# jimahlstrom/quisk

Measured on AMD Instinct MI355X. Metric: Mcomplex-samples/s through RXA chain, higher is better.
Workload: dtype f64; 1 GPU; 256 channels/GPU x 192 kHz IQ -> 48 kHz SSB RXA chain (shift + 561-tap resample/4 + adc meter + NBP nc 2048 + S meter + fixed AGC + agc meter + panel), 2^22 input samples per channel per step; meters=on, ingest=f64, channels_per_gpu=256, total_channels=256, dsp_size=256, parallelism=channel-sharded x1 (weak), no collective

## Files before the change

### quisk_amd/csrc/qh_fft.hpp

```cpp
#pragma once
#include <hip/hip_runtime.h>

namespace qh {

static constexpr double kThetaZeroMark = 8.0;


constexpr int NT = 256;

template <typename T> struct cplx_of;
template <> struct cplx_of<double> { using type = double2; };
template <> struct cplx_of<float>  { using type = float2; };
template <typename T> using cplx = typename cplx_of<T>::type;

template <typename T> __device__ __forceinline__ cplx<T> mk(T x, T y) { cplx<T> r; r.x = x; r.y = y; return r; }
template <typename C> __device__ __forceinline__ C cadd(C a, C b) { C r; r.x = a.x + b.x; r.y = a.y + b.y; return r; }
template <typename C> __device__ __forceinline__ C csub(C a, C b) { C r; r.x = a.x - b.x; r.y = a.y - b.y; return r; }
template <typename C> __device__ __forceinline__ C cmul(C a, C b)
{
    C r;
    r.x = a.x * b.x - a.y * b.y;
    r.y = a.x * b.y + a.y * b.x;
    return r;
}
__device__ __forceinline__ void lds_barrier()
{
    __builtin_amdgcn_fence(__ATOMIC_RELEASE, "workgroup", "local");
    __builtin_amdgcn_s_barrier();
    __builtin_amdgcn_fence(__ATOMIC_ACQUIRE, "workgroup", "local");
}

template <typename C> __device__ __forceinline__ C cconj(C a) { C r; r.x = a.x; r.y = -a.y; return r; }
template <bool INV, typename C> __device__ __forceinline__ C mul_mi(C a)
{
    C r;
    if (INV) { r.x = -a.y; r.y = a.x; } else { r.x = a.y; r.y = -a.x; }
    return r;
}

__device__ __forceinline__ constexpr double cos32(int a)
{
    constexpr double t[9] = { 1.0, 0.98078528040323044913, 0.92387953251128675613, 0.83146961230254523708,
                              0.70710678118654752440, 0.55557023301960222474, 0.38268343236508977173,
                              0.19509032201612826785, 0.0 };
    return t[a];
}

template <int R, int I, bool INV, typename C> __device__ __forceinline__ C mul_wconst(C a)
{
    using T = decltype(a.x);
    constexpr int A = I * (32 / R);
    if constexpr (A == 0) {
        return a;
    } else if constexpr (A == 8) {
        return mul_mi<INV>(a);
    } else if constexpr (A == 4) {
        const T s = (T)0.70710678118654752440;
        C r;
        if (INV) { r.x = (a.x - a.y) * s; r.y = (a.x + a.y) * s; }
        else     { r.x = (a.x + a.y) * s; r.y = (a.y - a.x) * s; }
        return r;
    } else if constexpr (A == 12) {
        const T s = (T)0.70710678118654752440;
        C r;
        if (INV) { r.x = -(a.x + a.y) * s; r.y = (a.x - a.y) * s; }
        else     { r.x = (a.y - a.x) * s;  r.y = -(a.x + a.y) * s; }
        return r;
    } else {
        constexpr double c = (A <= 8) ? cos32(A) : -cos32(16 - A);
        constexpr double s = (A <= 8) ? cos32(8 - A) : cos32(A - 8);
        C w;
        w.x = (T)c;
        w.y = INV ? (T)s : (T)(-s);
        return cmul(a, w);
    }
}

template <int R, bool INV, typename C> struct Dft {
    template <int I> static __device__ __forceinline__ void stage(C (&x)[R], C (&a)[R / 2], C (&b)[R / 2])
    {
        if constexpr (I < R / 2) {
            a[I] = cadd(x[I], x[I + R / 2]);
            b[I] = mul_wconst<R, I, INV>(csub(x[I], x[I + R / 2]));
            stage<I + 1>(x, a, b);
        }
    }
    static __device__ __forceinline__ void run(C (&x)[R])
    {
        C a[R / 2], b[R / 2];
        stage<0>(x, a, b);
        Dft<R / 2, INV, C>::run(a);
        Dft<R / 2, INV, C>::run(b);
#pragma unroll
        for (int q = 0; q < R / 2; q++) { x[2 * q] = a[q]; x[2 * q + 1] = b[q]; }
    }
};
template <bool INV, typename C> struct Dft<1, INV, C> { static __device__ __forceinline__ void run(C (&)[1]) {} };

__device__ __forceinline__ int lds_phys(int i) { return i + (i >> 4); }
template <int N> constexpr int lds_elems() { return N + N / 16; }

template <int R, typename C> __device__ __forceinline__ void apply_twiddle_powers(C (&x)[R], C w1)
{
    constexpr int H = R / 2 > 1 ? R / 2 : 1;
    C w[H + 1];
    w[1] = w1;
    x[1] = cmul(x[1], w1);
#pragma unroll
    for (int r = 2; r < R; r++) {
        int hi = 1;
        while (hi * 2 <= r) hi *= 2;
        const int lo = r - hi;
        C wr;
        if (hi < H || (hi == H && lo == 0)) {
            wr = (lo == 0) ? cmul(w[hi / 2], w[hi / 2]) : cmul(w[hi], w[lo]);
            w[r < H + 1 ? r : H] = wr;
        } else {
            wr = cmul(w[H], w[lo]);
        }
        x[r] = cmul(x[r], wr);
    }
}

template <int R, typename C> __device__ __forceinline__ void apply_twiddle_powers_lean(C (&x)[R], C w1)
{
    const C w2 = cmul(w1, w1);
    C we = w2, wo = w1;
    x[1] = cmul(x[1], wo);
#pragma unroll
    for (int r = 2; r < R; r++) {
        if (r & 1) { wo = cmul(wo, w2); x[r] = cmul(x[r], wo); }
        else { x[r] = cmul(x[r], we); if (r + 2 < R) we = cmul(we, w2); }
    }
}

template <int N, int R, int Ns, bool INV, typename C, bool LEAN = false>
__device__ __forceinline__ int stockham_butterfly(C (&x)[R], int j, C w1)
{
    int k = j & (Ns - 1);
    if constexpr (Ns > 1) { if constexpr (LEAN) apply_twiddle_powers_lean<R>(x, w1); else apply_twiddle_powers<R>(x, w1); }
    Dft<R, INV, C>::run(x);
    return (j - k) * R + k;
}

template <int Ns, bool INV, typename C>
__device__ __forceinline__ C pass_twiddle(const C *__restrict__ tw_pass, int j)
{
    C w = tw_pass[j & (Ns - 1)];
    return INV ? cconj(w) : w;
}

template <int N, int R, bool INV, typename C>
__device__ __forceinline__ void pass_regs_to_lds(C (&x)[R], C *lds)
{
    static_assert(R == N / NT, "first pass radix must equal N/NT");
    const int j = threadIdx.x;
    Dft<R, INV, C>::run(x);
    if constexpr (16 % R == 0) {
        C *p = lds + lds_phys(j * R);
#pragma unroll
        for (int r = 0; r < R; r++) p[r] = x[r];
    } else {
        static_assert(R % 16 == 0, "first pass radix: a divisor or a multiple of 16");
        C *p = lds + lds_phys(j * R);
#pragma unroll
        for (int r = 0; r < R; r++) p[r + r / 16] = x[r];
    }
}

template <int N, int R> struct PassGeom {
    static constexpr int NB = N / R;
    static constexpr int PER = (NB + NT - 1) / NT;
};

template <int N, int R, int Ns, bool INV, typename C>
__device__ __forceinline__ void pass_lds_to_lds(C *lds, const C (&w1)[PassGeom<N, R>::PER])
{
    constexpr int NB = PassGeom<N, R>::NB;
    constexpr int PER = PassGeom<N, R>::PER;
    C x[PER][R];
    int base[PER];
    static_assert(NB % 16 == 0, "pass geometry");
#pragma unroll
    for (int p = 0; p < PER; p++) {
        int j = threadIdx.x + p * NT;
        if (NB >= NT || j < NB) {
            const C *q = lds + lds_phys(j);
#pragma unroll
            for (int r = 0; r < R; r++) x[p][r] = q[r * (NB + NB / 16)];
        }
    }
#pragma unroll
    for (int p = 0; p < PER; p++) {
        int j = threadIdx.x + p * NT;
        if (NB >= NT || j < NB) base[p] = stockham_butterfly<N, R, Ns, INV>(x[p], j, w1[p]);
    }
    __syncthreads();
#pragma unroll
    for (int p = 0; p < PER; p++) {
        int j = threadIdx.x + p * NT;
        if (NB >= NT || j < NB) {
            if constexpr (Ns % 16 == 0) {
                C *q = lds + lds_phys(base[p]);
#pragma unroll
                for (int r = 0; r < R; r++) q[r * (Ns + Ns / 16)] = x[p][r];
            } else if constexpr (16 % (Ns * R) == 0) {
                C *q = lds + lds_phys(base[p]);
#pragma unroll
                for (int r = 0; r < R; r++) q[r * Ns] = x[p][r];
            } else {
#pragma unroll
                for (int r = 0; r < R; r++) lds[lds_phys(base[p] + r * Ns)] = x[p][r];
            }
        }
    }
}

template <int N, int R, bool INV, typename C>
__device__ __forceinline__ void pass_lds_to_regs(const C *lds, C (&x)[R], C w1)
{
    static_assert(R == N / NT, "last pass radix must equal N/NT");
    const int j = threadIdx.x;
    const C *q = lds + lds_phys(j);
#pragma unroll
    for (int r = 0; r < R; r++) x[r] = q[r * (NT + NT / 16)];
    stockham_butterfly<N, R, N / R, INV>(x, j, w1);
}

template <int N, bool INV, typename C> struct FftRR;

template <bool INV, typename C> struct FftRR<4096, INV, C> {
    struct Tw { C a[1], b; };
    static __device__ __forceinline__ Tw load(const C *__restrict__ tw) { return load_at(tw, threadIdx.x); }
    static __device__ __forceinline__ Tw load_at(const C *__restrict__ tw, int j)
    {
        Tw t;
        t.a[0] = pass_twiddle<16, INV>(tw, j);
        t.b = pass_twiddle<256, INV>(tw + 16, j);
        return t;
    }
    static __device__ __forceinline__ void first(C (&x)[16], C *lds) { pass_regs_to_lds<4096, 16, INV>(x, lds); }
    static __device__ __forceinline__ void rest(C *lds, C (&x)[16], const Tw &t)
    {
        __syncthreads();
        pass_lds_to_lds<4096, 16, 16, INV>(lds, t.a);
        __syncthreads();
        pass_lds_to_regs<4096, 16, INV>(lds, x, t.b);
    }
};

#ifndef QH_SPLIT_PAD
#define QH_SPLIT_PAD 2
#endif
#ifndef QH_SPLIT_SWIZZLE
#define QH_SPLIT_SWIZZLE 0
#endif
constexpr int split4096_lds_bytes(int scalar_bytes) { return (QH_SPLIT_SWIZZLE ? 4096 : 4096 + QH_SPLIT_PAD * 256) * scalar_bytes; }
template <bool INV, typename C> struct FftSplit4096 {
    using T = decltype(C{}.x);
    using Tw = typename FftRR<4096, INV, C>::Tw;
    static constexpr bool kSwizzle = QH_SPLIT_SWIZZLE != 0;
    template <int PHASE>
    static __device__ __forceinline__ void exchange_sw(C (&x)[16], T *lds, int j, int base)
    {
        const int m = j & 15;
        T *wb = PHASE == 1 ? lds + 16 * j : lds + (base - m);
        const T *rp = lds + 16 * (j >> 4) + (m ^ ((j >> 4) & 15));
#pragma unroll
        for (int r = 0; r < 16; r++) (PHASE == 1 ? wb : wb + 16 * r)[PHASE == 1 ? (r ^ m) : (m ^ r)] = x[r].x;
        __syncthreads();
#pragma unroll
        for (int r = 0; r < 16; r++) x[r].x = rp[256 * r];
        __syncthreads();
#pragma unroll
        for (int r = 0; r < 16; r++) (PHASE == 1 ? wb : wb + 16 * r)[PHASE == 1 ? (r ^ m) : (m ^ r)] = x[r].y;
        __syncthreads();
#pragma unroll
        for (int r = 0; r < 16; r++) x[r].y = rp[256 * r];
    }
    static constexpr int kPad = QH_SPLIT_PAD;
    static constexpr int kLdsBytes = split4096_lds_bytes((int)sizeof(T));
    static __device__ __forceinline__ int sphys(int i) { return i + (i >> 4) * kPad; }

    template <int WS, int RS, bool LB = false>
    static __device__ __forceinline__ void exchange(C (&x)[16], T *lds, int wbase, int rbase)
    {
        T *wp = lds + wbase;
        const T *rp = lds + rbase;
#pragma unroll
        for (int r = 0; r < 16; r++) wp[r * WS] = x[r].x;
        if (LB) lds_barrier(); else __syncthreads();
#pragma unroll
        for (int r = 0; r < 16; r++) x[r].x = rp[r * RS];
        if (LB) lds_barrier(); else __syncthreads();
#pragma unroll
        for (int r = 0; r < 16; r++) wp[r * WS] = x[r].y;
        if (LB) lds_barrier(); else __syncthreads();
#pragma unroll
        for (int r = 0; r < 16; r++) x[r].y = rp[r * RS];
    }

    static __device__ __forceinline__ void run(C (&x)[16], void *lds_raw, const Tw &t) { run_at(x, lds_raw, t, threadIdx.x); }
    template <bool LEAN = false>
    static __device__ __forceinline__ void run_at(C (&x)[16], void *lds_raw, const Tw &t, int j)
    {
        T *lds = reinterpret_cast<T *>(lds_raw);
        Dft<16, INV, C>::run(x);
        if constexpr (kSwizzle) exchange_sw<1>(x, lds, j, 0);
        else exchange<1, 256 + 16 * kPad>(x, lds, (16 + kPad) * j, sphys(j));
        const int base = stockham_butterfly<4096, 16, 16, INV, C, LEAN>(x, j, t.a[0]);
        __syncthreads();
        if constexpr (kSwizzle) exchange_sw<2>(x, lds, j, base);
        else exchange<16 + kPad, 256 + 16 * kPad>(x, lds, sphys(base), sphys(j));
        stockham_butterfly<4096, 16, 256, INV, C, LEAN>(x, j, t.b);
    }

    template <int D>
    static __device__ __forceinline__ void run_poly(C (&x)[16], void *lds_raw, const Tw &t)
    {
        static_assert(!INV && (D == 2 || D == 4 || D == 8), "forward transform of a decimating stage");
        constexpr int R3 = 16 / D;
        const int j = threadIdx.x;
        T *lds = reinterpret_cast<T *>(lds_raw);
        Dft<16, INV, C>::run(x);
        if constexpr (kSwizzle) exchange_sw<1>(x, lds, j, 0);
        else exchange<1, 256 + 16 * kPad>(x, lds, (16 + kPad) * j, sphys(j));
        const int base = stockham_butterfly<4096, 16, 16, INV>(x, j, t.a[0]);
        __syncthreads();
        if constexpr (kSwizzle) exchange_sw<2>(x, lds, j, base);
        else exchange<16 + kPad, 256 + 16 * kPad>(x, lds, sphys(base), sphys(j));
        C w[R3];
        w[1] = t.b;
#pragma unroll
        for (int s = 1; s < D; s <<= 1) w[1] = cmul(w[1], w[1]);
#pragma unroll
        for (int r = 2; r < R3; r++) w[r] = (r & 1) ? cmul(w[r - 1], w[1]) : cmul(w[r / 2], w[r / 2]);
        C y[16];
#pragma unroll
        for (int a = 0; a < D; a++) {
            C b[R3];
            b[0] = x[a];
#pragma unroll
            for (int r = 1; r < R3; r++) b[r] = cmul(x[a + D * r], w[r]);
            Dft<R3, INV, C>::run(b);
#pragma unroll
            for (int r = 0; r < R3; r++) y[r + R3 * a] = b[r];
        }
#pragma unroll
        for (int r = 0; r < 16; r++) x[r] = y[r];
    }
};

constexpr int kFft6kThreads = 384;
constexpr int kFft6kPad = 2;
constexpr int kFft6kLdsBytes = (6144 + 6144 / 16 * kFft6kPad) * 8;

template <bool INV, typename C> __device__ __forceinline__ void dft3(C &a, C &b, C &c)
{
    const double h = 0.86602540378443864676;
    const C t1 = cadd(b, c);
    C t2; t2.x = a.x - 0.5 * t1.x; t2.y = a.y - 0.5 * t1.y;
    const C d = csub(b, c);
    C t3;
    if (INV) { t3.x = -h * d.y; t3.y = h * d.x; } else { t3.x = h * d.y; t3.y = -h * d.x; }
    a = cadd(a, t1);
    b = cadd(t2, t3);
    c = csub(t2, t3);
}

template <int M, bool INV, typename C> __device__ __forceinline__ C mul_w24(C a)
{
    constexpr int m = M % 24;
    if constexpr (m == 0) return a;
    else if constexpr (m == 6) return mul_mi<INV>(a);
    else if constexpr (m == 12) { C r; r.x = -a.x; r.y = -a.y; return r; }
    else if constexpr (m == 18) return mul_mi<!INV>(a);
    else {
        constexpr double c15[7] = { 1.0, 0.96592582628906828675, 0.86602540378443864676, 0.70710678118654752440, 0.5,
                                    0.25881904510252076235, 0.0 };
        constexpr int q = m / 6, rem = m % 6;
        constexpr double cr = c15[rem], sr = c15[6 - rem];
        constexpr double co = q == 0 ? cr : q == 1 ? -sr : q == 2 ? -cr : sr;
        constexpr double si = q == 0 ? sr : q == 1 ? cr : q == 2 ? -sr : -cr;
        C w; w.x = co; w.y = INV ? si : -si;
        return cmul(a, w);
    }
}

template <bool INV, typename C> struct Dft24 {
    template <int N2> static __device__ __forceinline__ void tw(C (&y)[3][8])
    {
        if constexpr (N2 < 8) {
            y[1][N2] = mul_w24<N2, INV>(y[1][N2]);
            y[2][N2] = mul_w24<2 * N2, INV>(y[2][N2]);
            tw<N2 + 1>(y);
        }
    }
    static __device__ __forceinline__ void run(C (&x)[24])
    {
        C y[3][8];
#pragma unroll
        for (int n2 = 0; n2 < 8; n2++) {
            C a = x[n2], b = x[8 + n2], c = x[16 + n2];
            dft3<INV>(a, b, c);
            y[0][n2] = a; y[1][n2] = b; y[2][n2] = c;
        }
        tw<1>(y);
#pragma unroll
        for (int k1 = 0; k1 < 3; k1++) Dft<8, INV, C>::run(y[k1]);
#pragma unroll
        for (int k1 = 0; k1 < 3; k1++)
#pragma unroll
            for (int k2 = 0; k2 < 8; k2++) x[k1 + 3 * k2] = y[k1][k2];
// ... 3 lines not shown
template <typename C> __device__ __forceinline__ void apply_twiddle_powers24(C (&x)[24], C w1)
{
    const C w2 = cmul(w1, w1), w3 = cmul(w2, w1), w4 = cmul(w2, w2), w8 = cmul(w4, w4), w16 = cmul(w8, w8);
    const C w5 = cmul(w4, w1), w6 = cmul(w4, w2), w7 = cmul(w4, w3);
    x[1] = cmul(x[1], w1); x[2] = cmul(x[2], w2); x[3] = cmul(x[3], w3); x[4] = cmul(x[4], w4);
    x[5] = cmul(x[5], w5); x[6] = cmul(x[6], w6); x[7] = cmul(x[7], w7); x[8] = cmul(x[8], w8);
    x[9] = cmul(x[9], cmul(w8, w1)); x[10] = cmul(x[10], cmul(w8, w2)); x[11] = cmul(x[11], cmul(w8, w3));
    x[12] = cmul(x[12], cmul(w8, w4)); x[13] = cmul(x[13], cmul(w8, w5)); x[14] = cmul(x[14], cmul(w8, w6));
    x[15] = cmul(x[15], cmul(w8, w7)); x[16] = cmul(x[16], w16);
    x[17] = cmul(x[17], cmul(w16, w1)); x[18] = cmul(x[18], cmul(w16, w2)); x[19] = cmul(x[19], cmul(w16, w3));
    x[20] = cmul(x[20], cmul(w16, w4)); x[21] = cmul(x[21], cmul(w16, w5)); x[22] = cmul(x[22], cmul(w16, w6));
    x[23] = cmul(x[23], cmul(w16, w7));
}

template <bool INV> struct Fft6144 {
    using C = double2;
    static constexpr int kPad = kFft6kPad;
    static __device__ __forceinline__ int sphys(int i) { return i + (i >> 4) * kPad; }
    struct Tw { C mid, last; };
    static __device__ __forceinline__ Tw load(int t)
    {
        Tw w;
        double s, c;
        sincospi(-2.0 * (double)(t & 15) / 384.0, &s, &c);
        w.mid = make_double2(c, INV ? -s : s);
        sincospi(-2.0 * (double)t / 6144.0, &s, &c);
        w.last = make_double2(c, INV ? -s : s);
        return w;
    }
    static __device__ __forceinline__ void run(C (&x)[16], void *lds_raw, const Tw &tw, int t)
    {
        double *lds = reinterpret_cast<double *>(lds_raw);
        const bool mid = t < 256;
        Dft<16, INV, C>::run(x);
        C y[24];
        double *w1 = lds + (16 + kPad) * t;
        const double *r1 = lds + sphys(t);
#pragma unroll
        for (int r = 0; r < 16; r++) w1[r] = x[r].x;
        __syncthreads();
        if (mid) {
#pragma unroll
            for (int r = 0; r < 24; r++) y[r].x = r1[r * (256 + 16 * kPad)];
        }
        __syncthreads();
#pragma unroll
        for (int r = 0; r < 16; r++) w1[r] = x[r].y;
        __syncthreads();
        const int k = t & 15, u = t >> 4;
        double *w2 = lds + (384 + 24 * kPad) * u + k;
        if (mid) {
#pragma unroll
            for (int r = 0; r < 24; r++) y[r].y = r1[r * (256 + 16 * kPad)];
            apply_twiddle_powers24(y, tw.mid);
            Dft24<INV, C>::run(y);
        }
        __syncthreads();
        if (mid) {
#pragma unroll
            for (int r = 0; r < 24; r++) w2[r * (16 + kPad)] = y[r].x;
        }
        __syncthreads();
        const double *r2 = lds + sphys(t);
#pragma unroll
        for (int r = 0; r < 16; r++) x[r].x = r2[r * (384 + 24 * kPad)];
        __syncthreads();
        if (mid) {
#pragma unroll
            for (int r = 0; r < 24; r++) w2[r * (16 + kPad)] = y[r].y;
        }
        __syncthreads();
#pragma unroll
        for (int r = 0; r < 16; r++) x[r].y = r2[r * (384 + 24 * kPad)];
        apply_twiddle_powers<16>(x, tw.last);
        Dft<16, INV, C>::run(x);
    }
};

template <int N, bool INV, typename C> struct TileFft {
    static constexpr bool kSplit = N == 4096 && sizeof(C) == 16;
    static constexpr int kLdsBytes = kSplit ? split4096_lds_bytes(8) : lds_elems<N>() * (int)sizeof(C);
    using Tw = typename FftRR<N, INV, C>::Tw;
    static __device__ __forceinline__ Tw load(const C *__restrict__ tw) { return FftRR<N, INV, C>::load(tw); }
    static __device__ __forceinline__ void run(C (&x)[N / NT], void *lds, const Tw &t)
    {
        if constexpr (kSplit) {
            FftSplit4096<INV, C>::run(x, lds, t);
        } else {
            FftRR<N, INV, C>::first(x, reinterpret_cast<C *>(lds));
            FftRR<N, INV, C>::rest(reinterpret_cast<C *>(lds), x, t);
        }
    }
    template <int D> static __device__ __forceinline__ void run_poly(C (&x)[N / NT], void *lds, const Tw &t)
    {
        static_assert(kSplit, "polyphase plan: the fp64 4096-point transform");
        FftSplit4096<INV, C>::template run_poly<D>(x, lds, t);
    }
};

template <bool INV, typename C> struct FftRR<2048, INV, C> {
    struct Tw { C a[2], b[1], c; };
    static __device__ __forceinline__ Tw load(const C *__restrict__ tw)
    {
        Tw t;
        t.a[0] = pass_twiddle<8, INV>(tw, threadIdx.x);
        t.a[1] = pass_twiddle<8, INV>(tw, threadIdx.x + NT);
        t.b[0] = pass_twiddle<32, INV>(tw + 8, threadIdx.x);
        t.c = pass_twiddle<256, INV>(tw + 40, threadIdx.x);
        return t;
    }
    static __device__ __forceinline__ void first(C (&x)[8], C *lds) { pass_regs_to_lds<2048, 8, INV>(x, lds); }
    static __device__ __forceinline__ void rest(C *lds, C (&x)[8], const Tw &t)
    {
        __syncthreads();
        pass_lds_to_lds<2048, 4, 8, INV>(lds, t.a);
        __syncthreads();
        pass_lds_to_lds<2048, 8, 32, INV>(lds, t.b);
        __syncthreads();
        pass_lds_to_regs<2048, 8, INV>(lds, x, t.c);
    }
};

template <bool INV, typename C> struct FftRR<1024, INV, C> {
    struct Tw { C a[1], b[1], c[1], d; };
    static __device__ __forceinline__ Tw load(const C *__restrict__ tw)
    {
        Tw t;
        t.a[0] = pass_twiddle<4, INV>(tw, threadIdx.x);
        t.b[0] = pass_twiddle<16, INV>(tw + 4, threadIdx.x);
        t.c[0] = pass_twiddle<64, INV>(tw + 20, threadIdx.x);
        t.d = pass_twiddle<256, INV>(tw + 84, threadIdx.x);
        return t;
    }
    static __device__ __forceinline__ void first(C (&x)[4], C *lds) { pass_regs_to_lds<1024, 4, INV>(x, lds); }
    static __device__ __forceinline__ void rest(C *lds, C (&x)[4], const Tw &t)
    {
        __syncthreads();
        pass_lds_to_lds<1024, 4, 4, INV>(lds, t.a);
        __syncthreads();
        pass_lds_to_lds<1024, 4, 16, INV>(lds, t.b);
        __syncthreads();
        pass_lds_to_lds<1024, 4, 64, INV>(lds, t.c);
        __syncthreads();
        pass_lds_to_regs<1024, 4, INV>(lds, x, t.d);
    }
};

template <bool INV, typename C> struct FftRR<512, INV, C> {
    struct Tw { C a[1], b[1], c; };
    static __device__ __forceinline__ Tw load(const C *__restrict__ tw)
    {
        Tw t;
        t.a[0] = pass_twiddle<2, INV>(tw, threadIdx.x);
        t.b[0] = pass_twiddle<32, INV>(tw + 2, threadIdx.x);
        t.c = pass_twiddle<256, INV>(tw + 34, threadIdx.x);
        return t;
    }
    static __device__ __forceinline__ void first(C (&x)[2], C *lds) { pass_regs_to_lds<512, 2, INV>(x, lds); }
    static __device__ __forceinline__ void rest(C *lds, C (&x)[2], const Tw &t)
    {
        __syncthreads();
        pass_lds_to_lds<512, 16, 2, INV>(lds, t.a);
        __syncthreads();
        pass_lds_to_lds<512, 8, 32, INV>(lds, t.b);
        __syncthreads();
        pass_lds_to_regs<512, 2, INV>(lds, x, t.c);
    }
};

template <bool INV, typename C> struct FftRR<8192, INV, C> {
    struct Tw { C a[4], b; };
    static __device__ __forceinline__ Tw load(const C *__restrict__ tw)
    {
        Tw t;
#pragma unroll
        for (int p = 0; p < 4; p++) t.a[p] = pass_twiddle<32, INV>(tw, threadIdx.x + p * NT);
        t.b = pass_twiddle<256, INV>(tw + 32, threadIdx.x);
        return t;
    }
    static __device__ __forceinline__ void first(C (&x)[32], C *lds) { pass_regs_to_lds<8192, 32, INV>(x, lds); }
    static __device__ __forceinline__ void rest(C *lds, C (&x)[32], const Tw &t)
    {
        __syncthreads();
        pass_lds_to_lds<8192, 8, 32, INV>(lds, t.a);
        __syncthreads();
        pass_lds_to_regs<8192, 32, INV>(lds, x, t.b);
    }
};

}
```

### quisk_amd/csrc/qh_osfir.hpp

```cpp
#pragma once
#include "qh_fft.hpp"
#include "qh_wave.hpp"
#include "qh_ingest.hpp"
#include "qh_egress.hpp"

namespace qh {


struct EpiParam {
    double a, b, c, d;
};

template <typename T> struct OsfirArgs {
    const cplx<T> *in;
    const cplx<T> *hist;
    cplx<T> *hist_next;
    cplx<T> *out;
    const cplx<T> *mask;
    const cplx<T> *tw_fwd;
    const cplx<T> *tw_inv;
    const unsigned long long *nco_phase;
    const unsigned long long *nco_dphase;
    const double2 *nco_step;
    const EpiParam *epi;
// ... 38 lines not shown
    long long amlv_stride;
    const double *amlv_cin;
    long long amlv_cstride;
    const double *amlv_pw;
    int amlv_shift;
};


__device__ __forceinline__ double fm_audio_at(const double *a_local, const double *cin, const double *pw, int shift, double gain, long long g)
{
    const long long t = g >> shift;
    const int k = (int)(g - (t << shift));
    return gain * __builtin_fma(-cin[t], pw[k], a_local[g]);
}

template <typename T> __device__ __forceinline__ void sincos_turns(unsigned long long ph, T &c, T &s);
template <> __device__ __forceinline__ void sincos_turns<double>(unsigned long long ph, double &c, double &s)
{
    double t = (double)(ph >> 11) * (1.0 / 9007199254740992.0);
    sincospi(2.0 * t, &s, &c);
}
template <> __device__ __forceinline__ void sincos_turns<float>(unsigned long long ph, float &c, float &s)
{
    double t = (double)(ph >> 11) * (1.0 / 9007199254740992.0);
    double sd, cd;
    sincospi(2.0 * t, &sd, &cd);
    c = (float)cd; s = (float)sd;
}

template <typename T, int E>
__device__ __forceinline__ unsigned load_tile(cplx<T> (&x)[E], const cplx<T> *__restrict__ in,
                                              const cplx<T> *__restrict__ hist, int hist_len, int n_in, int g0)
{
    using C = cplx<T>;
    const C *hsafe = hist ? hist : in;
    const int hlen = hist ? hist_len : 0;
    const int last = n_in - 1;
    unsigned okbits = 0;
#pragma unroll
    for (int r = 0; r < E; r++) {
        const int g = g0 + (int)threadIdx.x + r * NT;
        const int gi = g < 0 ? 0 : (g > last ? last : g);
        const int gh = g + hlen < 0 ? 0 : g + hlen;
        const C *p = g >= 0 ? in + gi : hsafe + (g < 0 ? gh : 0);
        const bool ok = g >= 0 ? g <= last : (g + hlen >= 0);
        okbits |= (ok ? 1u : 0u) << r;
        x[r] = *p;
    }
    return okbits;
}

#ifndef QH_XCD_SWIZZLE
#define QH_XCD_SWIZZLE 1
#endif
__device__ __forceinline__ void xcd_tile_map(int ntiles, int &chan_slot, int &tile)
{
    const unsigned G = gridDim.x, lin = blockIdx.x;
#if QH_XCD_SWIZZLE
    const unsigned c = lin & 7u, k = lin >> 3, q = G >> 3, rem = G & 7u;
    const unsigned gt = c * q + (c < rem ? c : rem) + k;
#else
    const unsigned gt = lin;
    (void)G;
#endif
    chan_slot = (int)(gt / (unsigned)ntiles);
    tile = (int)(gt - (unsigned)chan_slot * (unsigned)ntiles);
}

template <typename T, int NFFT, int D, bool METER = false> constexpr int osfir_lds_bytes()
{
    constexpr int a = TileFft<NFFT, false, cplx<T>>::kLdsBytes, b = TileFft<NFFT / D, true, cplx<T>>::kLdsBytes;
    constexpr int m = METER ? NT / 64 * 2 * 64 * 9 * 8 : 0;
    return (a > b ? a : b) > m ? (a > b ? a : b) : m;
}
template <typename T, int NFFT, int U> constexpr int osfir_interp_lds_bytes()
{
    constexpr int a = TileFft<NFFT / U, false, cplx<T>>::kLdsBytes, b = TileFft<NFFT, true, cplx<T>>::kLdsBytes;
    return a > b ? a : b;
}

#ifndef QH_MASK_BATCH
#define QH_MASK_BATCH 8
#endif
#ifndef QH_OSFIR_WAVES_F64_D1
#define QH_OSFIR_WAVES_F64_D1 4
#endif
#ifndef QH_OSFIR_WAVES_F64
#define QH_OSFIR_WAVES_F64 3
#endif
#ifndef QH_OSFIR_WAVES_F64_OUTMIX
#define QH_OSFIR_WAVES_F64_OUTMIX 3
#endif
template <typename T, int D, bool OUTMIX = false, int NFFT = 4096> constexpr int osfir_min_waves()
{
    if (NFFT >= 8192) return sizeof(T) == 8 ? 1 : 2;
    return sizeof(T) == 8 ? (D == 1 ? QH_OSFIR_WAVES_F64_D1 : OUTMIX ? QH_OSFIR_WAVES_F64_OUTMIX : QH_OSFIR_WAVES_F64) : 4;
}

#ifdef QH_OSFIR_PROBE
__device__ long long g_osfir_probe[16];
#define QH_OPROBE(slot) do { if (blockIdx.x == 7 * 8 && threadIdx.x == 0) g_osfir_probe[slot] = clock64(); } while (0)
#else
#define QH_OPROBE(slot) do { } while (0)
#endif


template <int CTRL> __device__ __forceinline__ double dpp_mov_d(double v)
{
    int lo = __double2loint(v), hi = __double2hiint(v);
    lo = __builtin_amdgcn_mov_dpp(lo, CTRL, 0xf, 0xf, false);
    hi = __builtin_amdgcn_mov_dpp(hi, CTRL, 0xf, 0xf, false);
    return __hiloint2double(hi, lo);
}
constexpr int kMeterLdsDoublesPerWave = 2 * 64 * 9;

__device__ __forceinline__ double max_nn(double a, double b)
{
    double r;
    asm("v_max_f64 %0, %1, %2" : "=v"(r) : "v"(a), "v"(b));
    return r;
}

template <typename C, int E>
__device__ __forceinline__ void meter_tap(const C (&x)[E], int r0, double wlane, double *lds_wave, double2 *dst, int wave, int lane, int wstride = -1)
{
    const int ws = wstride < 0 ? E - r0 : wstride;
    const int wr = (lane >> 3) * 9 + (lane & 7);
    const double *rd = lds_wave + lane * 9;
#pragma unroll
    for (int g = 0; g < E / 8; g++) {
        if (8 * (g + 1) <= r0) continue;
#pragma unroll
        for (int k = 0; k < 8; k++) {
            const C v = x[8 * g + k];
            double m2 = (double)v.x * (double)v.x;
            m2 = __builtin_fma((double)v.y, (double)v.y, m2);
            lds_wave[k * 72 + wr] = m2 * wlane;
            lds_wave[64 * 9 + k * 72 + wr] = m2;
        }
        __builtin_amdgcn_fence(__ATOMIC_RELEASE, "wavefront");
        __builtin_amdgcn_wave_barrier();
        __builtin_amdgcn_fence(__ATOMIC_ACQUIRE, "wavefront");
        double sum = rd[0], mx = rd[64 * 9];
#pragma unroll
        for (int k = 1; k < 8; k++) { sum += rd[k]; mx = max_nn(mx, rd[64 * 9 + k]); }
        sum += dpp_mov_d<0xB1>(sum); mx = max_nn(mx, dpp_mov_d<0xB1>(mx));
        sum += dpp_mov_d<0x4E>(sum); mx = max_nn(mx, dpp_mov_d<0x4E>(mx));
        sum += dpp_mov_d<0x141>(sum); mx = max_nn(mx, dpp_mov_d<0x141>(mx));
        const int r = 8 * g + (lane >> 3);
        if ((lane & 7) == 0 && r >= r0) dst[wave * ws + (r - r0)] = make_double2(sum, mx);
        __builtin_amdgcn_wave_barrier();
    }
}

template <typename T, int NFFT, int D, bool MIX, bool PACKED = false, bool METER = false, bool OUTMIX = false, bool EGRESS = false, bool POLY = false,
          int DET = 0, bool PAIR = false>
__global__ __launch_bounds__(NT, (osfir_min_waves<T, D, OUTMIX, NFFT>())) void osfir_kernel(OsfirArgs<T> a)
{
    using C = cplx<T>;
    constexpr int E = NFFT / NT;
    constexpr int NOUT = NFFT / D;
    constexpr int EO = E / D;
    static_assert(E % D == 0 && EO >= 1, "decimation must divide NFFT/256");
    static_assert(NOUT >= 2 * NT, "NFFT/D must be >= 512");
    static_assert(E <= 32, "validity bits are kept in one word");
    using Fwd = TileFft<NFFT, false, C>;
    using Inv = TileFft<NOUT, true, C>;
    extern __shared__ __align__(16) unsigned char smem[];
    void *lds = smem;

    const int t = threadIdx.x;
    int tile, slot;
    xcd_tile_map(a.ntiles, slot, tile);
    const int ch = PAIR ? a.chan_list[2 * slot] : a.chan_list ? a.chan_list[slot] : slot;
    const int ch_b = PAIR ? a.chan_list[2 * slot + 1] : ch;
    const C *in = a.in + (long long)ch * a.in_stride;
    const C *hist = a.hist ? a.hist + (long long)ch * a.hist_stride : nullptr;
    const int g0 = a.off - a.P + tile * (D * a.Lout);

    QH_OPROBE(0);
    C x[E];
    const bool interior = (g0 >= 0) && (g0 + NFFT <= a.n_in);
    if constexpr (PACKED) {
        const long long base = a.pk.first_offset + (long long)ch * a.pk.chan_stride + (long long)g0 * a.pk.record_stride;
        const bool fast = interior && a.pk.records_per_frame == 0 &&
                          base + (long long)(NFFT - 1) * a.pk.record_stride + 8 <= a.pk.total_bytes;
        if (fast) {
            const unsigned char *p = a.pk_src + base + (long long)t * a.pk.record_stride;
            const long long step = (long long)NT * a.pk.record_stride;
#pragma unroll
            for (int r = 0; r < E; r++) x[r] = decode_packed_at<T>(p + r * step, a.pk.sel_re, a.pk.sel_im, a.pk.gain);
        } else if (interior) {
#pragma unroll
            for (int r = 0; r < E; r++) x[r] = decode_packed<T>(a.pk_src, a.pk, ch, (long long)(g0 + t + r * NT));
        } else {
#pragma unroll
            for (int r = 0; r < E; r++) {
                const int g = g0 + t + r * NT;
                if (g >= 0) x[r] = g < a.n_in ? decode_packed<T>(a.pk_src, a.pk, ch, (long long)g) : mk<T>(0, 0);
                else x[r] = (hist && g + a.hist_len >= 0) ? hist[g + a.hist_len] : mk<T>(0, 0);
            }
        }
    } else if constexpr (PAIR) {
        static_assert(!MIX && !METER && !OUTMIX && !EGRESS && DET == 0, "pairs ride on a plain stage (any fold: a real filter acts on the two parts alike)");
        const C *in_b = a.in + (long long)ch_b * a.in_stride;
        const C *hist_b = a.hist ? a.hist + (long long)ch_b * a.hist_stride : nullptr;
        if (a.fmdc_a) {
            const double *aa = a.fmdc_a + (long long)ch * a.fmdc_stride, *ab = a.fmdc_a + (long long)ch_b * a.fmdc_stride;
            const double *ca = a.fmdc_cin + (long long)ch * a.fmdc_cstride, *cb = a.fmdc_cin + (long long)ch_b * a.fmdc_cstride;
            const double ga = a.fmdc_gain[ch], gb = a.fmdc_gain[ch_b];
            if (interior) {
#pragma unroll
                for (int r = 0; r < E; r++) {
                    const long long g = (long long)g0 + t + r * NT;
                    const long long tl = g >> a.fmdc_shift;
                    const double pw = a.fmdc_pw[(int)(g - (tl << a.fmdc_shift))];
                    x[r] = mk<T>((T)(ga * __builtin_fma(-ca[tl], pw, aa[g])), (T)(gb * __builtin_fma(-cb[tl], pw, ab[g])));
                }
            } else {
                auto fetch = [&](const double *src, const double *cin, double gain, const C *h, int g) -> T {
                    if (g >= 0) return g < a.n_in ? (T)fm_audio_at(src, cin, a.fmdc_pw, a.fmdc_shift, gain, g) : (T)0;
                    return (h && g + a.hist_len >= 0) ? h[g + a.hist_len].x : (T)0;
                };
#pragma unroll
                for (int r = 0; r < E; r++) {
                    const int g = g0 + t + r * NT;
                    x[r] = mk<T>(fetch(aa, ca, ga, hist, g), fetch(ab, cb, gb, hist_b, g));
                }
            }
        } else if (a.amlv_a) {
            const double *aa = a.amlv_a + (long long)ch * a.amlv_stride, *ab = a.amlv_a + (long long)ch_b * a.amlv_stride;
            const double2 *ca = reinterpret_cast<const double2 *>(a.amlv_cin) + (long long)ch * a.amlv_cstride;
            const double2 *cb = reinterpret_cast<const double2 *>(a.amlv_cin) + (long long)ch_b * a.amlv_cstride;
            const double *pwR = a.amlv_pw, *pwI = a.amlv_pw + (1 << a.amlv_shift);
            auto fetch = [&](const double *src, const double2 *cin, const C *h, int g) -> T {
                if (g >= 0) {
                    if (g >= a.n_in) return (T)0;
                    const int tl = g >> a.amlv_shift, k = g - (tl << a.amlv_shift);
                    const double2 c = cin[tl];
                    return (T)(src[g] + __builtin_fma(c.y, pwI[k], -c.x * pwR[k]));
                }
                return (h && g + a.hist_len >= 0) ? h[g + a.hist_len].x : (T)0;
            };
            if (interior) {
#pragma unroll
                for (int r = 0; r < E; r++) {
                    const int g = g0 + t + r * NT;
                    const int tl = g >> a.amlv_shift, k = g - (tl << a.amlv_shift);
                    const double2 c0 = ca[tl], c1 = cb[tl];
                    const double wR = pwR[k], wI = pwI[k];
                    x[r] = mk<T>((T)(aa[g] + __builtin_fma(c0.y, wI, -c0.x * wR)), (T)(ab[g] + __builtin_fma(c1.y, wI, -c1.x * wR)));
                }
            } else {
#pragma unroll
                for (int r = 0; r < E; r++) {
                    const int g = g0 + t + r * NT;
                    x[r] = mk<T>(fetch(aa, ca, hist, g), fetch(ab, cb, hist_b, g));
                }
            }
        } else if (interior) {
            const C *p = in + g0 + t, *pb = in_b + g0 + t;
#pragma unroll
            for (int r = 0; r < E; r++) x[r] = mk<T>(p[r * NT].x, pb[r * NT].x);
        } else {
            auto fetch = [&](const C *src, const C *h, int g) -> T {
                if (g >= 0) return g < a.n_in ? src[g].x : (T)0;
                return (h && g + a.hist_len >= 0) ? h[g + a.hist_len].x : (T)0;
            };
#pragma unroll
            for (int r = 0; r < E; r++) {
                const int g = g0 + t + r * NT;
                x[r] = mk<T>(fetch(in, hist, g), fetch(in_b, hist_b, g));
            }
        }
    } else if (interior) {
        const C *p = in + g0 + t;
#pragma unroll
        for (int r = 0; r < E; r++) x[r] = p[r * NT];
    } else {
        const unsigned ok = load_tile<T, E>(x, in, hist, a.hist_len, a.n_in, g0);
#pragma unroll
        for (int r = 0; r < E; r++)
            if (!((ok >> r) & 1u)) x[r] = mk<T>(0, 0);
    }
    if constexpr (MIX) {
        C rot;
        sincos_turns<T>(a.nco_phase[ch] + a.nco_dphase[ch] * (unsigned long long)(long long)(g0 + t), rot.x, rot.y);
        const double2 st = a.nco_step[ch];
        const C step = mk<T>((T)st.x, (T)st.y);
        if (interior) {
#pragma unroll
            for (int r = 0; r < E; r++) { x[r] = cmul(x[r], rot); rot = cmul(rot, step); }
        } else {
#pragma unroll
            for (int r = 0; r < E; r++) {
                if (g0 + t + r * NT >= 0) x[r] = cmul(x[r], rot);
                rot = cmul(rot, step);
            }
        }
    }

    if constexpr (METER) {
        static_assert(D == 1 && !MIX && !PACKED, "meters ride on a plain D = 1 stage");
        static_assert(NT / 64 * kMeterLdsDoublesPerWave * 8 <= osfir_lds_bytes<T, NFFT, D, true>(), "meter blocks overlay the exchange image");
        meter_tap<C, E>(x, a.P >> 8, a.meter_w[t & 63], reinterpret_cast<double *>(lds) + (t >> 6) * kMeterLdsDoublesPerWave,
                        a.meter_in + (long long)ch * a.meter_stride + (long long)tile * (a.Lout >> 6), t >> 6, t & 63);
        __syncthreads();
    }

    QH_OPROBE(1);
    if constexpr (POLY) Fwd::template run_poly<D>(x, lds, Fwd::load(a.tw_fwd));
    else Fwd::run(x, lds, Fwd::load(a.tw_fwd));
    QH_OPROBE(2);

    const C *mask = a.mask + (long long)ch * a.mask_stride;
    C z[EO];
#pragma unroll
    for (int i = 0; i < EO; i++) {
        C acc = cmul(x[i], mask[t + NT * i]);
#pragma unroll
        for (int q = 1; q < D; q++) acc = cadd(acc, cmul(x[i + EO * q], mask[t + NT * (i + EO * q)]));
        z[i] = acc;
        if (((i + 1) * D) % QH_MASK_BATCH == 0) __builtin_amdgcn_sched_barrier(0);
    }

    QH_OPROBE(3);
    __syncthreads();
    Inv::run(z, lds, Inv::load(a.tw_inv));
    QH_OPROBE(4);
    if constexpr (METER) {
        __syncthreads();
        int t2 = t;
        asm volatile("" : "+v"(t2));
        meter_tap<C, EO>(z, a.P >> 8, a.meter_w[t2 & 63], reinterpret_cast<double *>(lds) + (t2 >> 6) * kMeterLdsDoublesPerWave,
                         a.meter_out + (long long)ch * a.meter_stride + (long long)tile * (a.Lout >> 6), t2 >> 6, t2 & 63);
    }

    if constexpr (OUTMIX) {
        static_assert(!MIX, "one oscillator");
        const double2 tr = a.tile_rot[(long long)ch * a.ntiles + tile];
        const double2 lr = a.lane_rot[(long long)ch * NT + t];
        const double2 st = a.nco_step[ch];
        C rot = cmul(mk<T>((T)tr.x, (T)tr.y), mk<T>((T)lr.x, (T)lr.y));
        const C step = mk<T>((T)st.x, (T)st.y);
#pragma unroll
        for (int i = 0; i < EO; i++) {
            z[i] = cmul(z[i], rot);
            if (i + 1 < EO) rot = cmul(rot, step);
        }
    }

    C *out = a.out + (long long)ch * a.out_stride + a.out_offset;
    const int j0 = a.P / D;
    EpiParam ep;
    if (a.epi) ep = a.epi[ch]; else { ep.a = 1; ep.b = 0; ep.c = 0; ep.d = 1; }
    if constexpr (PAIR) {
        C *out_b = a.out + (long long)ch_b * a.out_stride + a.out_offset;
        EpiParam eb = ep;
        if (a.epi) eb = a.epi[ch_b];
#pragma unroll
        for (int i = 0; i < EO; i++) {
            const int rel = t + NT * i - j0;
            const long long m = (long long)tile * a.Lout + rel;
            if (rel >= 0 && rel < a.Lout && m < a.n_out) {
                const T ya = z[i].x, yb = z[i].y;
                const T ia = a.pair_im0 ? (T)0 : ya, ib = a.pair_im0 ? (T)0 : yb;
                out[m] = mk<T>((T)ep.a * ya + (T)ep.b * ia, (T)ep.c * ya + (T)ep.d * ia);
                out_b[m] = mk<T>((T)eb.a * yb + (T)eb.b * ib, (T)eb.c * yb + (T)eb.d * ib);
            }
        }
    } else if constexpr (DET == 3) {
        static_assert(D == 1 && NT == 256 && NFFT == 4096 && !EGRESS && !METER && !PAIR && !OUTMIX, "the leveller's tap rides on a plain 4096-point stage");
        constexpr int R0 = 8, NR = 8;
        const int lane = t & 63, wv = t >> 6;
        const bool lf = a.det_lf[ch] != 0;
        double *sv = reinterpret_cast<double *>(lds);
        double *red = sv + NR * NT;
        static_assert((NR * NT + 2 * 4 * NR + 2) * 8 <= osfir_lds_bytes<T, NFFT, D, false>(), "the leveller's scans fit the exchange image");
        __syncthreads();
        int lane2 = lane;
        asm volatile("" : "+v"(lane2));
        PoleScan sR, sI;
        sR.m1 = a.det_mp[0][0]; sR.m2 = a.det_mp[0][1]; sR.m4 = a.det_mp[0][2]; sR.m8 = a.det_mp[0][3];
        sI.m1 = a.det_mp[1][0]; sI.m2 = a.det_mp[1][1]; sI.m4 = a.det_mp[1][2]; sI.m8 = a.det_mp[1][3];
        sR.pa = a.det_scan[lane2]; sR.pb = a.det_scan[64 + lane2]; sR.pw = a.det_scan[128 + lane2];
        sI.pa = a.det_scan[192 + lane2]; sI.pb = a.det_scan[256 + lane2]; sI.pw = a.det_scan[320 + lane2];
        const long long m0 = (long long)tile * a.Lout + t;
#pragma unroll
        for (int r = 0; r < NR; r++) {
            const long long m = m0 + NT * r;
            C v;
            v.x = (T)ep.a * z[R0 + r].x + (T)ep.b * z[R0 + r].y;
            v.y = (T)ep.c * z[R0 + r].x + (T)ep.d * z[R0 + r].y;
            const double mag = m < a.n_out ? sqrt((double)v.x * (double)v.x + (double)v.y * (double)v.y) : 0.0;
            const double vR = scan_pole_dpp(a.det_g[0] * mag, sR), vI = scan_pole_dpp(a.det_g[1] * mag, sI);
            sv[r * NT + t] = lf ? mag + (vI - vR) : mag;
            if (lane2 == 63) { red[(4 * r + wv) * 2] = vR; red[(4 * r + wv) * 2 + 1] = vI; }
            if (m == (long long)a.n_out - 1) { red[2 * 4 * NR] = vR; red[2 * 4 * NR + 1] = vI; }
            __builtin_amdgcn_sched_barrier(0);
        }
        __syncthreads();
        const double m64R = ipow_d(a.det_m[0], 64), m64I = ipow_d(a.det_m[1], 64);
        double cR = 0.0, cI = 0.0;
#pragma unroll
        for (int r = 0; r < NR; r++) {
            double kR = 0.0, kI = 0.0;
#pragma unroll
            for (int w = 0; w < 4; w++) {
                if (w == wv) { kR = cR; kI = cI; }
                cR = __builtin_fma(cR, m64R, red[(4 * r + w) * 2]);
                cI = __builtin_fma(cI, m64I, red[(4 * r + w) * 2 + 1]);
            }
            const long long m = m0 + NT * r;
            if (m < a.n_out) {
                const double cR_here = sR.pw * kR, cI_here = sI.pw * kI;
                a.det_out[(long long)ch * a.det_stride + a.out_offset + m] = lf ? sv[r * NT + t] + (cI_here - cR_here) : sv[r * NT + t];
                if (m == (long long)a.n_out - 1) { a.det_last[2 * ch] = red[2 * 4 * NR] + cR_here; a.det_last[2 * ch + 1] = red[2 * 4 * NR + 1] + cI_here; }
            }
            __builtin_amdgcn_sched_barrier(0);
        }
        if (t == 0) {
            double *o = a.det_sum + ((long long)ch * a.det_sum_stride + tile) * 2;
            o[0] = lf ? cR : 0.0; o[1] = lf ? cI : 0.0;
        }
    } else if (a.pick <= 1) {
        double acc0 = 0.0, acc1 = 0.0;
#pragma unroll
        for (int i = 0; i < EO; i++) {
            const int rel = t + NT * i - j0;
            const long long m = (long long)tile * a.Lout + rel;
            double mag = 0.0;
            if (rel >= 0 && rel < a.Lout && m < a.n_out) {
                C v;
                v.x = (T)ep.a * z[i].x + (T)ep.b * z[i].y;
                v.y = (T)ep.c * z[i].x + (T)ep.d * z[i].y;
                if constexpr (DET == 1) {
                    double th = atan2((double)v.y, (double)v.x) * (1.0 / 6.2831853071795864);
                    if (v.x == (T)0 && v.y == (T)0) th = kThetaZeroMark;
// ... 340 lines not shown
```

Measured before the change: 142,400 Mcomplex-samples/s.

## Prefetch mask and oscillator loads inside FFT; use LDS-only barriers for f64 OUTMIX tile

For the fp64 4096-point OUTMIX stage with decimation 2 or 4, the kernel now starts loading the spectral mask halfway through the forward FFT through a mid-transform hook. The mask multiply runs as a sliding-window software pipeline. The lane rotation and inverse twiddles are loaded during that pipeline, and the per-tile rotation, NCO step and epilogue parameters are hoisted to the kernel start. Full __syncthreads in the FFT exchanges are replaced by LDS-only fence barriers, which hides global load latency behind compute but raises register pressure and could lower occupancy.

```diff
diff --git a/quisk_amd/csrc/qh_fft.hpp b/quisk_amd/csrc/qh_fft.hpp
--- a/quisk_amd/csrc/qh_fft.hpp
+++ b/quisk_amd/csrc/qh_fft.hpp
@@ -29,6 +29,11 @@
     __builtin_amdgcn_s_barrier();
     __builtin_amdgcn_fence(__ATOMIC_ACQUIRE, "workgroup", "local");
 }
+template <bool LB> __device__ __forceinline__ void tile_barrier()
+{
+    if constexpr (LB) lds_barrier(); else __syncthreads();
+}
+struct NoMidHook { __device__ __forceinline__ void operator()() const {} };
 
 template <typename C> __device__ __forceinline__ C cconj(C a) { C r; r.x = a.x; r.y = -a.y; return r; }
 template <bool INV, typename C> __device__ __forceinline__ C mul_mi(C a)
@@ -173,7 +178,7 @@
     static constexpr int PER = (NB + NT - 1) / NT;
 };
 
-template <int N, int R, int Ns, bool INV, typename C>
+template <int N, int R, int Ns, bool INV, typename C, bool LB = false>
 __device__ __forceinline__ void pass_lds_to_lds(C *lds, const C (&w1)[PassGeom<N, R>::PER])
 {
     constexpr int NB = PassGeom<N, R>::NB;
@@ -195,7 +200,7 @@
         int j = threadIdx.x + p * NT;
         if (NB >= NT || j < NB) base[p] = stockham_butterfly<N, R, Ns, INV>(x[p], j, w1[p]);
     }
-    __syncthreads();
+    tile_barrier<LB>();
 #pragma unroll
     for (int p = 0; p < PER; p++) {
         int j = threadIdx.x + p * NT;
@@ -240,11 +245,11 @@
         return t;
     }
     static __device__ __forceinline__ void first(C (&x)[16], C *lds) { pass_regs_to_lds<4096, 16, INV>(x, lds); }
-    static __device__ __forceinline__ void rest(C *lds, C (&x)[16], const Tw &t)
-    {
-        __syncthreads();
-        pass_lds_to_lds<4096, 16, 16, INV>(lds, t.a);
-        __syncthreads();
+    template <bool LB = false> static __device__ __forceinline__ void rest(C *lds, C (&x)[16], const Tw &t)
+    {
+        tile_barrier<LB>();
+        pass_lds_to_lds<4096, 16, 16, INV, C, LB>(lds, t.a);
+        tile_barrier<LB>();
         pass_lds_to_regs<4096, 16, INV>(lds, x, t.b);
     }
 };
@@ -300,23 +305,25 @@
         for (int r = 0; r < 16; r++) x[r].y = rp[r * RS];
     }
 
-    static __device__ __forceinline__ void run(C (&x)[16], void *lds_raw, const Tw &t) { run_at(x, lds_raw, t, threadIdx.x); }
-    template <bool LEAN = false>
-    static __device__ __forceinline__ void run_at(C (&x)[16], void *lds_raw, const Tw &t, int j)
+    template <bool LB = false, typename Mid = NoMidHook>
+    static __device__ __forceinline__ void run(C (&x)[16], void *lds_raw, const Tw &t, Mid &&mid = Mid()) { run_at<false, LB>(x, lds_raw, t, threadIdx.x, mid); }
+    template <bool LEAN = false, bool LB = false, typename Mid = NoMidHook>
+    static __device__ __forceinline__ void run_at(C (&x)[16], void *lds_raw, const Tw &t, int j, Mid &&mid = Mid())
     {
         T *lds = reinterpret_cast<T *>(lds_raw);
         Dft<16, INV, C>::run(x);
         if constexpr (kSwizzle) exchange_sw<1>(x, lds, j, 0);
-        else exchange<1, 256 + 16 * kPad>(x, lds, (16 + kPad) * j, sphys(j));
+        else exchange<1, 256 + 16 * kPad, LB>(x, lds, (16 + kPad) * j, sphys(j));
         const int base = stockham_butterfly<4096, 16, 16, INV, C, LEAN>(x, j, t.a[0]);
-        __syncthreads();
+        mid();
+        tile_barrier<LB>();
         if constexpr (kSwizzle) exchange_sw<2>(x, lds, j, base);
-        else exchange<16 + kPad, 256 + 16 * kPad>(x, lds, sphys(base), sphys(j));
+        else exchange<16 + kPad, 256 + 16 * kPad, LB>(x, lds, sphys(base), sphys(j));
         stockham_butterfly<4096, 16, 256, INV, C, LEAN>(x, j, t.b);
     }
 
-    template <int D>
-    static __device__ __forceinline__ void run_poly(C (&x)[16], void *lds_raw, const Tw &t)
+    template <int D, bool LB = false, typename Mid = NoMidHook>
+    static __device__ __forceinline__ void run_poly(C (&x)[16], void *lds_raw, const Tw &t, Mid &&mid = Mid())
     {
         static_assert(!INV && (D == 2 || D == 4 || D == 8), "forward transform of a decimating stage");
         constexpr int R3 = 16 / D;
@@ -324,11 +331,12 @@
         T *lds = reinterpret_cast<T *>(lds_raw);
         Dft<16, INV, C>::run(x);
         if constexpr (kSwizzle) exchange_sw<1>(x, lds, j, 0);
-        else exchange<1, 256 + 16 * kPad>(x, lds, (16 + kPad) * j, sphys(j));
+        else exchange<1, 256 + 16 * kPad, LB>(x, lds, (16 + kPad) * j, sphys(j));
         const int base = stockham_butterfly<4096, 16, 16, INV>(x, j, t.a[0]);
-        __syncthreads();
+        mid();
+        tile_barrier<LB>();
         if constexpr (kSwizzle) exchange_sw<2>(x, lds, j, base);
-        else exchange<16 + kPad, 256 + 16 * kPad>(x, lds, sphys(base), sphys(j));
+        else exchange<16 + kPad, 256 + 16 * kPad, LB>(x, lds, sphys(base), sphys(j));
         C w[R3];
         w[1] = t.b;
 #pragma unroll
@@ -498,19 +506,22 @@
     static constexpr int kLdsBytes = kSplit ? split4096_lds_bytes(8) : lds_elems<N>() * (int)sizeof(C);
     using Tw = typename FftRR<N, INV, C>::Tw;
     static __device__ __forceinline__ Tw load(const C *__restrict__ tw) { return FftRR<N, INV, C>::load(tw); }
-    static __device__ __forceinline__ void run(C (&x)[N / NT], void *lds, const Tw &t)
+    template <bool LB = false, typename Mid = NoMidHook>
+    static __device__ __forceinline__ void run(C (&x)[N / NT], void *lds, const Tw &t, Mid &&mid = Mid())
     {
         if constexpr (kSplit) {
-            FftSplit4096<INV, C>::run(x, lds, t);
+            FftSplit4096<INV, C>::template run<LB>(x, lds, t, mid);
         } else {
             FftRR<N, INV, C>::first(x, reinterpret_cast<C *>(lds));
-            FftRR<N, INV, C>::rest(reinterpret_cast<C *>(lds), x, t);
-        }
-    }
-    template <int D> static __device__ __forceinline__ void run_poly(C (&x)[N / NT], void *lds, const Tw &t)
+            mid();
+            FftRR<N, INV, C>::template rest<LB>(reinterpret_cast<C *>(lds), x, t);
+        }
+    }
+    template <int D, bool LB = false, typename Mid = NoMidHook>
+    static __device__ __forceinline__ void run_poly(C (&x)[N / NT], void *lds, const Tw &t, Mid &&mid = Mid())
     {
         static_assert(kSplit, "polyphase plan: the fp64 4096-point transform");
-        FftSplit4096<INV, C>::template run_poly<D>(x, lds, t);
+        FftSplit4096<INV, C>::template run_poly<D, LB>(x, lds, t, mid);
     }
 };
 
@@ -526,13 +537,13 @@
         return t;
     }
     static __device__ __forceinline__ void first(C (&x)[8], C *lds) { pass_regs_to_lds<2048, 8, INV>(x, lds); }
-    static __device__ __forceinline__ void rest(C *lds, C (&x)[8], const Tw &t)
-    {
-        __syncthreads();
-        pass_lds_to_lds<2048, 4, 8, INV>(lds, t.a);
-        __syncthreads();
-        pass_lds_to_lds<2048, 8, 32, INV>(lds, t.b);
-        __syncthreads();
+    template <bool LB = false> static __device__ __forceinline__ void rest(C *lds, C (&x)[8], const Tw &t)
+    {
+        tile_barrier<LB>();
+        pass_lds_to_lds<2048, 4, 8, INV, C, LB>(lds, t.a);
+        tile_barrier<LB>();
+        pass_lds_to_lds<2048, 8, 32, INV, C, LB>(lds, t.b);
+        tile_barrier<LB>();
         pass_lds_to_regs<2048, 8, INV>(lds, x, t.c);
     }
 };
@@ -549,15 +560,15 @@
         return t;
     }
     static __device__ __forceinline__ void first(C (&x)[4], C *lds) { pass_regs_to_lds<1024, 4, INV>(x, lds); }
-    static __device__ __forceinline__ void rest(C *lds, C (&x)[4], const Tw &t)
-    {
-        __syncthreads();
-        pass_lds_to_lds<1024, 4, 4, INV>(lds, t.a);
-        __syncthreads();
-        pass_lds_to_lds<1024, 4, 16, INV>(lds, t.b);
-        __syncthreads();
-        pass_lds_to_lds<1024, 4, 64, INV>(lds, t.c);
-        __syncthreads();
+    template <bool LB = false> static __device__ __forceinline__ void rest(C *lds, C (&x)[4], const Tw &t)
+    {
+        tile_barrier<LB>();
+        pass_lds_to_lds<1024, 4, 4, INV, C, LB>(lds, t.a);
+        tile_barrier<LB>();
+        pass_lds_to_lds<1024, 4, 16, INV, C, LB>(lds, t.b);
+        tile_barrier<LB>();
+        pass_lds_to_lds<1024, 4, 64, INV, C, LB>(lds, t.c);
+        tile_barrier<LB>();
         pass_lds_to_regs<1024, 4, INV>(lds, x, t.d);
     }
 };
@@ -573,13 +584,13 @@
         return t;
     }
     static __device__ __forceinline__ void first(C (&x)[2], C *lds) { pass_regs_to_lds<512, 2, INV>(x, lds); }
-    static __device__ __forceinline__ void rest(C *lds, C (&x)[2], const Tw &t)
-    {
-        __syncthreads();
-        pass_lds_to_lds<512, 16, 2, INV>(lds, t.a);
-        __syncthreads();
-        pass_lds_to_lds<512, 8, 32, INV>(lds, t.b);
-        __syncthreads();
+    template <bool LB = false> static __device__ __forceinline__ void rest(C *lds, C (&x)[2], const Tw &t)
+    {
+        tile_barrier<LB>();
+        pass_lds_to_lds<512, 16, 2, INV, C, LB>(lds, t.a);
+        tile_barrier<LB>();
+        pass_lds_to_lds<512, 8, 32, INV, C, LB>(lds, t.b);
+        tile_barrier<LB>();
         pass_lds_to_regs<512, 2, INV>(lds, x, t.c);
     }
 };
@@ -595,11 +606,11 @@
         return t;
     }
     static __device__ __forceinline__ void first(C (&x)[32], C *lds) { pass_regs_to_lds<8192, 32, INV>(x, lds); }
-    static __device__ __forceinline__ void rest(C *lds, C (&x)[32], const Tw &t)
-    {
-        __syncthreads();
-        pass_lds_to_lds<8192, 8, 32, INV>(lds, t.a);
-        __syncthreads();
+    template <bool LB = false> static __device__ __forceinline__ void rest(C *lds, C (&x)[32], const Tw &t)
+    {
+        tile_barrier<LB>();
+        pass_lds_to_lds<8192, 8, 32, INV, C, LB>(lds, t.a);
+        tile_barrier<LB>();
         pass_lds_to_regs<8192, 32, INV>(lds, x, t.b);
     }
 };
diff --git a/quisk_amd/csrc/qh_osfir.hpp b/quisk_amd/csrc/qh_osfir.hpp
--- a/quisk_amd/csrc/qh_osfir.hpp
+++ b/quisk_amd/csrc/qh_osfir.hpp
@@ -144,6 +144,15 @@
 #ifndef QH_MASK_BATCH
 #define QH_MASK_BATCH 8
 #endif
+#ifndef QH_TILE_LB
+#define QH_TILE_LB 1
+#endif
+#ifndef QH_MASK_BATCH_D4
+#define QH_MASK_BATCH_D4 10
+#endif
+#ifndef QH_MASK_AHEAD
+#define QH_MASK_AHEAD 8
+#endif
 #ifndef QH_OSFIR_WAVES_F64_D1
 #define QH_OSFIR_WAVES_F64_D1 4
 #endif
@@ -239,6 +248,15 @@
     const C *in = a.in + (long long)ch * a.in_stride;
     const C *hist = a.hist ? a.hist + (long long)ch * a.hist_stride : nullptr;
     const int g0 = a.off - a.P + tile * (D * a.Lout);
+
+    constexpr bool LB = QH_TILE_LB && sizeof(T) == 8 && NFFT == 4096 && OUTMIX && (D == 2 || D == 4) && !METER && !EGRESS && DET == 0 && !PAIR;
+    [[maybe_unused]] double2 tr_top, st_top;
+    [[maybe_unused]] EpiParam ep_top;
+    if constexpr (LB) {
+        tr_top = a.tile_rot[(long long)ch * a.ntiles + tile];
+        st_top = a.nco_step[ch];
+        if (a.epi) ep_top = a.epi[ch]; else { ep_top.a = 1; ep_top.b = 0; ep_top.c = 0; ep_top.d = 1; }
+    }
 
     QH_OPROBE(0);
     C x[E];
@@ -370,25 +388,72 @@
         __syncthreads();
     }
 
+    constexpr int kWindow = D == 4 && !PACKED ? QH_MASK_BATCH_D4 : QH_MASK_BATCH, kMaskAhead = QH_MASK_AHEAD;
+    static_assert(!LB || (kMaskAhead >= 1 && kMaskAhead <= kWindow && kWindow <= E), "mask window");
+    const C *mask;
+    [[maybe_unused]] C m[E];
+    auto mask_load = [&](int k) { m[k] = mask[t + NT * (k / D + EO * (k % D))]; };
+
     QH_OPROBE(1);
-    if constexpr (POLY) Fwd::template run_poly<D>(x, lds, Fwd::load(a.tw_fwd));
-    else Fwd::run(x, lds, Fwd::load(a.tw_fwd));
+    if constexpr (LB) {
+        mask = a.mask + (long long)ch * a.mask_stride;
+        auto mid_fwd = [&]() {
+#pragma unroll
+            for (int k = 0; k < kMaskAhead; k++) mask_load(k);
+        };
+        if constexpr (POLY) Fwd::template run_poly<D, LB>(x, lds, Fwd::load(a.tw_fwd), mid_fwd);
+        else Fwd::template run<LB>(x, lds, Fwd::load(a.tw_fwd), mid_fwd);
+    } else {
+        if constexpr (POLY) Fwd::template run_poly<D>(x, lds, Fwd::load(a.tw_fwd));
+        else Fwd::run(x, lds, Fwd::load(a.tw_fwd));
+    }
     QH_OPROBE(2);
-
-    const C *mask = a.mask + (long long)ch * a.mask_stride;
+    if constexpr (!LB) mask = a.mask + (long long)ch * a.mask_stride;
+
     C z[EO];
-#pragma unroll
-    for (int i = 0; i < EO; i++) {
-        C acc = cmul(x[i], mask[t + NT * i]);
-#pragma unroll
-        for (int q = 1; q < D; q++) acc = cadd(acc, cmul(x[i + EO * q], mask[t + NT * (i + EO * q)]));
-        z[i] = acc;
-        if (((i + 1) * D) % QH_MASK_BATCH == 0) __builtin_amdgcn_sched_barrier(0);
-    }
-
-    QH_OPROBE(3);
-    __syncthreads();
-    Inv::run(z, lds, Inv::load(a.tw_inv));
+    [[maybe_unused]] C rot_top;
+    if constexpr (!LB) {
+#pragma unroll
+        for (int i = 0; i < EO; i++) {
+            C acc = cmul(x[i], mask[t + NT * i]);
+#pragma unroll
+            for (int q = 1; q < D; q++) acc = cadd(acc, cmul(x[i + EO * q], mask[t + NT * (i + EO * q)]));
+            z[i] = acc;
+            if (((i + 1) * D) % QH_MASK_BATCH == 0) __builtin_amdgcn_sched_barrier(0);
+        }
+
+        QH_OPROBE(3);
+        __syncthreads();
+        Inv::run(z, lds, Inv::load(a.tw_inv));
+    } else {
+        typename Inv::Tw tw_inv;
+        double2 lr;
+#pragma unroll
+        for (int k = kMaskAhead; k < kWindow; k++) mask_load(k);
+        __builtin_amdgcn_sched_barrier(0);
+#pragma unroll
+        for (int k = 0; k < E; k++) {
+            const int i = k / D, q = k % D;
+            if (k > 0) {
+                __builtin_amdgcn_sched_barrier(0);
+                if (k + kWindow - 1 < E) mask_load(k + kWindow - 1);
+            }
+            const C pr = cmul(x[i + EO * q], m[k]);
+            z[i] = q == 0 ? pr : cadd(z[i], pr);
+            if (k == kMaskAhead - 1) {
+                __builtin_amdgcn_sched_barrier(0);
+                lr = a.lane_rot[(long long)ch * NT + t];
+                tw_inv = Inv::load(a.tw_inv);
+            }
+        }
+        __builtin_amdgcn_sched_barrier(0);
+        rot_top = cmul(mk<T>((T)tr_top.x, (T)tr_top.y), mk<T>((T)lr.x, (T)lr.y));
+        asm volatile("" : "+v"(rot_top.x), "+v"(rot_top.y));
+
+        QH_OPROBE(3);
+        tile_barrier<LB>();
+        Inv::template run<LB>(z, lds, tw_inv);
+    }
     QH_OPROBE(4);
     if constexpr (METER) {
         __syncthreads();
@@ -400,11 +465,17 @@
 
     if constexpr (OUTMIX) {
         static_assert(!MIX, "one oscillator");
-        const double2 tr = a.tile_rot[(long long)ch * a.ntiles + tile];
-        const double2 lr = a.lane_rot[(long long)ch * NT + t];
-        const double2 st = a.nco_step[ch];
-        C rot = cmul(mk<T>((T)tr.x, (T)tr.y), mk<T>((T)lr.x, (T)lr.y));
-        const C step = mk<T>((T)st.x, (T)st.y);
+        C rot, step;
+        if constexpr (LB) {
+            rot = rot_top;
+            step = mk<T>((T)st_top.x, (T)st_top.y);
+        } else {
+            const double2 tr = a.tile_rot[(long long)ch * a.ntiles + tile];
+            const double2 lr = a.lane_rot[(long long)ch * NT + t];
+            const double2 st = a.nco_step[ch];
+            rot = cmul(mk<T>((T)tr.x, (T)tr.y), mk<T>((T)lr.x, (T)lr.y));
+            step = mk<T>((T)st.x, (T)st.y);
+        }
 #pragma unroll
         for (int i = 0; i < EO; i++) {
             z[i] = cmul(z[i], rot);
@@ -415,7 +486,8 @@
     C *out = a.out + (long long)ch * a.out_stride + a.out_offset;
     const int j0 = a.P / D;
     EpiParam ep;
-    if (a.epi) ep = a.epi[ch]; else { ep.a = 1; ep.b = 0; ep.c = 0; ep.d = 1; }
+    if constexpr (LB) ep = ep_top;
+    else if (a.epi) ep = a.epi[ch]; else { ep.a = 1; ep.b = 0; ep.c = 0; ep.d = 1; }
     if constexpr (PAIR) {
         C *out_b = a.out + (long long)ch_b * a.out_stride + a.out_offset;
         EpiParam eb = ep;
```

New measurement: 143,600 Mcomplex-samples/s, median of 6. No clear change (+0.9%).
